# AIRI-Institute/nablaDFT

Hardware: AMD Instinct MI355X
Metric: conformer-steps/sec (fwd+bwd) + MAE(E,F) vs CPU reference (higher is better)
Workload: dtype f32 (dense products >= 192 tiles: f32 values split exactly into 3 bf16 pieces, 6 MFMA piece products, f32 accumulate; non-finite operands give NaN where plain f32 gives inf); 1 GPU; PaiNN-OC (nablaDFT/painn_pyg, config/model/painn-oc.yaml: F=128 L=6 R=100 rc=5A K=100) energy+forces train step incl. neighbour list, L1+L2 loss, grad all-reduce, clip 5.0, AdamW lr 5e-4; synthetic ~42-atom drug-like conformers, 2048 conformers/GPU/step; conformers_per_gpu=2048, edges_last_step=1737976, parallelism=dp1

## Files before the change

### include/nablaq.h

```cpp
#ifndef NABLAQ_H
#define NABLAQ_H
#include <stddef.h>
#include <stdint.h>

#ifdef __cplusplus
extern "C" {
#endif

#define NQ_OK 0
#define NQ_ERR_HIP 1
#define NQ_ERR_ARG 2
#define NQ_ERR_MOL_TOO_LARGE 3
#define NQ_ERR_WORKSPACE 4
#define NQ_ERR_NO_EDGES 5

#define NQ_ABI_VERSION 17

typedef struct nq_painn_cfg {
  int32_t hidden_channels;
  int32_t num_layers;
  int32_t num_rbf;
  int32_t num_elements;
  int32_t max_neighbors;
  int32_t envelope_exponent;
// ... 267 lines not shown
int nq_eq_layernorm_forward(const float* x, int64_t x_stride, const float* weight, const float* bias, int64_t rows, int32_t W, float eps, float* y, int64_t y_stride,
                            float* stats, void* stream);
size_t nq_eq_layernorm_scratch_floats(int64_t rows, int32_t W);
int nq_eq_layernorm_backward(const float* x, int64_t x_stride, const float* weight, const float* grad_y, int64_t g_stride, const float* stats, int64_t rows, int32_t W,
                             float* grad_x, int64_t gx_stride, float* grad_weight, float* grad_bias, float* scratch, void* stream);
int nq_eq_norm_sh_forward(const float* x, const float* w0, const float* b0, const float* affine_weight, const float* balance_weight, int64_t N, int32_t lmax,
                          int32_t C, float eps, float* y, float* stats, void* stream);
size_t nq_eq_norm_sh_scratch_floats(int64_t N, int32_t lmax, int32_t C);
int nq_eq_norm_sh_backward(const float* x, const float* w0, const float* affine_weight, const float* balance_weight, const float* grad_y, const float* stats,
                           int64_t N, int32_t lmax, int32_t C, float* grad_x, float* grad_w0, float* grad_b0, float* grad_affine_weight, float* scratch,
                           void* stream);
int nq_eq_logits_forward(const float* x, const float* alpha_dot, int64_t E, int32_t H, int32_t A, float* z, void* stream);
size_t nq_eq_logits_scratch_floats(int64_t E, int32_t H, int32_t A);
int nq_eq_logits_backward(const float* x, const float* alpha_dot, const float* grad_z, int64_t E, int32_t H, int32_t A, float* grad_x, float* grad_alpha_dot,
                          float* scratch, void* stream);
int nq_eq_softmax_forward(const float* z, const int32_t* ptr, int64_t N, int32_t H, float* out, void* stream);
int nq_eq_softmax_backward(const float* y, const float* grad_y, const int32_t* ptr, int64_t N, int32_t H, float* grad_z, void* stream);
int nq_eq_head_scale(int32_t nseg, const int32_t* rows, const float* const* x, const float* const* grad, const float* alpha, int64_t E, int32_t H, int32_t V,
                     float* const* out, float* grad_alpha, void* stream);
int nq_eq_scale(const float* x, const float* row_scale, const int32_t* row_index, const float* coef_scale, int64_t N, int32_t I, int32_t C, float* out, void* stream);

int nq_loss_l1_l2(const float* energy, const float* y, int32_t B, const float* forces, const float* f_target, int32_t N, float coef_e,
                  float coef_f, float* loss, float* grad_energy, float* grad_forces, void* stream);
int nq_loss_mse(const float* energy, const float* y, int32_t B, const float* forces, const float* f_target, int32_t N, float coef_e,
                float coef_f, float* loss, float* grad_energy, float* grad_forces, void* stream);
int nq_adamw_step(float* params, const float* grads, float* exp_avg, float* exp_avg_sq, size_t count, float max_norm, float lr,
                  float beta1, float beta2, float eps, float weight_decay, int32_t step, float* scratch, void* stream);

void nq_profile_enable(int32_t on);
int nq_profile_read(char* names_host, int32_t name_stride, double* total_ms_host, int64_t* counts_host, int32_t cap);
int nq_profile_read2(char* names_host, int32_t name_stride, double* total_ms_host, int64_t* counts_host, double* flops_host, int32_t cap);

void nq_set_gemm_variant(int32_t variant);
void nq_gemm_splitk_release(void);
int nq_gemm_splitk_state(void* stream, uint64_t* ptr, uint64_t* floats, int32_t* captured, int32_t* retired);

int nq_linear_forward(const float* A, const float* W, const float* bias, float* C, float* C_silu, int32_t M, int32_t N, int32_t K,
                      void* stream);
int nq_linear_forward_act(const float* A, const float* W, float* C, float* C_act, const float* resid, float alpha, float beta, int32_t M, int32_t N,
                          int32_t K, void* stream);
int nq_linear_forward_res(const float* A, const float* W, const float* aux, float alpha, float* C, int32_t M, int32_t N, int32_t K, void* stream);
int nq_bf16_pack(const float* W, int32_t N, int32_t K, void* Wb, void* WbT, void* stream);
int nq_linear_forward_bf16(const float* A, const void* Wb, float* C, float* C_act, const float* resid, float alpha, float beta, int32_t M, int32_t N,
                           int32_t K, void* stream);
int nq_linear_input_grad_bf16(const float* G, const void* WbT, float* C, int32_t M, int32_t N, int32_t K, int32_t accumulate, void* stream);
size_t nq_weight_grad_bf16_scratch_bytes(int64_t rows, int32_t N, int32_t K);
int nq_linear_weight_grad_bf16(const float* G, const float* X, float* gW, int64_t rows, int32_t N, int32_t K, void* scratch, void* stream);
int nq_linear_forward_bf16_out(const void* A, int32_t a_bf16, const void* Wb, void* pre_bf16, void* act, int32_t act_bf16, const float* resid, float alpha,
                               float beta, int32_t M, int32_t N, int32_t K, void* stream);
int nq_linear_weight_grad_bf16_x(const float* G, const void* X_bf16, float* gW, int64_t rows, int32_t N, int32_t K, void* scratch, void* stream);
int nq_gn_ssilu_backward_bf16(const void* z_bf16, const float* g, float scale, int64_t n, float* out, void* stream);
int nq_linear_input_grad(const float* G, const float* W, float* C, int32_t M, int32_t N, int32_t K, int32_t accumulate, void* stream);
int nq_linear_input_grad_epi(const float* G, const float* W, float* C, int32_t M, int32_t N, int32_t K, const float* aux, float alpha, float beta, int32_t mode,
                             void* stream);
int nq_linear_input_grad_bf16_epi(const float* G, const void* WbT, float* C, int32_t M, int32_t N, int32_t K, const float* aux, float alpha, float beta,
                                  int32_t mode, void* stream);
size_t nq_column_sum_scratch_floats(int64_t rows, int32_t cols);
int nq_column_sum(const float* A, int64_t rows, int32_t cols, int64_t lda, float* out, float* scratch, void* stream);
size_t nq_weight_grad_scratch_floats(int64_t rows, int32_t N, int32_t K);
int nq_linear_weight_grad(const float* G, const float* X, float* gW, int64_t rows, int32_t N, int32_t K, float* scratch, void* stream);
int nq_linear_weight_grad_bias(const float* G, const float* X, float* gW, float* gb, int64_t rows, int32_t N, int32_t K, float* scratch, void* stream);

int nq_rccl_available(void);
int nq_rccl_unique_id(void* id128);
int nq_rccl_comm_create(const void* id128, int32_t world, int32_t rank, void** comm);
int nq_rccl_comm_destroy(void* comm);
// ... 164 lines not shown
```

### nabladft_amd/_lib.py

```python
import ctypes as C
import os

import torch

_HERE = os.path.dirname(os.path.abspath(__file__))
LIB_PATH = os.environ.get("NABLAQ_LIB") or os.path.join(_HERE, "libnablaq.so")
ABI_VERSION = 17

NQ_OK, NQ_ERR_HIP, NQ_ERR_ARG, NQ_ERR_MOL_TOO_LARGE, NQ_ERR_WORKSPACE, NQ_ERR_NO_EDGES = range(6)


class NablaqError(RuntimeError):
    def __init__(self, code, msg):
        super().__init__(f"libnablaq error {code}: {msg}")
        self.code = code


class PainnCfg(C.Structure):
    _fields_ = [("hidden_channels", C.c_int32), ("num_layers", C.c_int32), ("num_rbf", C.c_int32),
                ("num_elements", C.c_int32), ("max_neighbors", C.c_int32), ("envelope_exponent", C.c_int32),
                ("cutoff", C.c_double), ("rbf_coeff", C.c_float), ("filter_mode", C.c_int32), ("rbf_type", C.c_int32), ("reserved", C.c_int32)]


class SchnetCfg(C.Structure):
# ... 134 lines not shown
    "nq_es_graph_fill": (C.c_int, [_P, _P, _P, _I32, _D, _I32, _P, _P, _P, _P, _P]),
    "nq_es_frames": (C.c_int, [_P, _I32, _P, _P]),
    "nq_es_wigner": (C.c_int, [_P, _I32, _P, _P, _P, _P, _I32, _I32, _I32, _P, _P, _P]),
    "nq_es_smearing": (C.c_int, [_P, _I64, _I32, _P, _F, _P, _P]),
    "nq_rowop": (C.c_int, [_P, _I64, _P, _I64, _P, _P, _I64, _I64, _I32, _I32, _I32, _I32, _I32, _P]),
    "nq_rowop_blocks": (C.c_int, [_P, _I64, _P, _I64, _P, _I32, _I32, _P, _P, _I64, _I32, _I32, _I32, _I32, _I32, _P]),
    "nq_s2_activation_blocks": (C.c_int, [_P, _P, _I32, _I32, _I32, _I64, _I32, _P, _P, _P, _P, _I32, _P]),
    "nq_column_sum_scratch_floats": (_SZ, [_I64, _I32]),
    "nq_column_sum": (C.c_int, [_P, _I64, _I32, _I64, _P, _P, _P]),
    "nq_es_rotate": (C.c_int, [_P, _I64, _P, _I64, _P, _I32, _P, _P, _I32, _I32, _I64, _P, _I32, _I32, _I32, _P]),
    "nq_es_rotate_back": (C.c_int, [_P, _I64, _I32, _P, _P, _I32, _I32, _P, _P, _P, _P, _I64, _P, _I32, _I32, _I32, _P]),
    "nq_eq_layernorm_forward": (C.c_int, [_P, _I64, _P, _P, _I64, _I32, _F, _P, _I64, _P, _P]),
    "nq_eq_layernorm_scratch_floats": (_SZ, [_I64, _I32]),
    "nq_eq_layernorm_backward": (C.c_int, [_P, _I64, _P, _P, _I64, _P, _I64, _I32, _P, _I64, _P, _P, _P, _P]),
    "nq_eq_norm_sh_forward": (C.c_int, [_P, _P, _P, _P, _P, _I64, _I32, _I32, _F, _P, _P, _P]),
    "nq_eq_norm_sh_scratch_floats": (_SZ, [_I64, _I32, _I32]),
    "nq_eq_norm_sh_backward": (C.c_int, [_P, _P, _P, _P, _P, _P, _I64, _I32, _I32, _P, _P, _P, _P, _P, _P]),
    "nq_eq_logits_forward": (C.c_int, [_P, _P, _I64, _I32, _I32, _P, _P]),
    "nq_eq_logits_scratch_floats": (_SZ, [_I64, _I32, _I32]),
    "nq_eq_logits_backward": (C.c_int, [_P, _P, _P, _I64, _I32, _I32, _P, _P, _P, _P]),
    "nq_eq_softmax_forward": (C.c_int, [_P, _P, _I64, _I32, _P, _P]),
    "nq_eq_softmax_backward": (C.c_int, [_P, _P, _P, _I64, _I32, _P, _P]),
    "nq_eq_head_scale": (C.c_int, [_I32, _P, _P, _P, _P, _I64, _I32, _I32, _P, _P, _P]),
    "nq_eq_scale": (C.c_int, [_P, _P, _P, _P, _I64, _I32, _I32, _P, _P]),
    "nq_loss_l1_l2": (C.c_int, [_P, _P, _I32, _P, _P, _I32, _F, _F, _P, _P, _P, _P]),
    "nq_loss_mse": (C.c_int, [_P, _P, _I32, _P, _P, _I32, _F, _F, _P, _P, _P, _P]),
    "nq_adamw_step": (C.c_int, [_P, _P, _P, _P, _SZ, _F, _F, _F, _F, _F, _F, _I32, _P, _P]),
    "nq_profile_enable": (None, [_I32]),
    "nq_profile_read": (C.c_int, [C.c_char_p, _I32, C.POINTER(C.c_double), C.POINTER(C.c_int64), _I32]),
    "nq_profile_read2": (C.c_int, [C.c_char_p, _I32, C.POINTER(C.c_double), C.POINTER(C.c_int64), C.POINTER(C.c_double), _I32]),
    "nq_set_gemm_variant": (None, [_I32]),
    "nq_gemm_splitk_release": (None, []),
    "nq_gemm_splitk_state": (C.c_int, [_P, C.POINTER(C.c_uint64), C.POINTER(C.c_uint64), C.POINTER(C.c_int32), C.POINTER(C.c_int32)]),
    "nq_linear_forward": (C.c_int, [_P, _P, _P, _P, _P, _I32, _I32, _I32, _P]),
    "nq_linear_input_grad": (C.c_int, [_P, _P, _P, _I32, _I32, _I32, _I32, _P]),
    "nq_weight_grad_scratch_floats": (_SZ, [_I64, _I32, _I32]),
    "nq_linear_weight_grad": (C.c_int, [_P, _P, _P, _I64, _I32, _I32, _P, _P]),
    "nq_linear_weight_grad_bias": (C.c_int, [_P, _P, _P, _P, _I64, _I32, _I32, _P, _P]),
    "nq_rccl_available": (C.c_int, []),
    "nq_rccl_unique_id": (C.c_int, [_P]),
    "nq_rccl_comm_create": (C.c_int, [_P, _I32, _I32, C.POINTER(C.c_void_p)]),
    "nq_rccl_comm_destroy": (C.c_int, [_P]),
    "nq_rccl_comm_count": (C.c_int, [_P, C.POINTER(C.c_int32)]),
    "nq_allreduce": (C.c_int, [_P, _SZ, _P, _P]),
    "nq_allreduce_mean": (C.c_int, [_P, _SZ, _P, _P]),
    "nq_rccl_broadcast": (C.c_int, [_P, _SZ, _I32, _P, _P]),
    "nq_lbfgs_state_bytes": (_SZ, [_I32, _I32, _I32]),
    "nq_lbfgs_state_layout": (C.c_int, [_I32, _I32, _I32, C.POINTER(_SZ)]),
    "nq_lbfgs_init": (C.c_int, [_P, _SZ, _P, _I32, _I32, _I32, _P, _I32, _P, C.POINTER(C.c_int32), _P]),
    "nq_lbfgs_step": (C.c_int, [_P, _I32, _I32, _I32, _I32, _P, _I32, _P, _P, _D, _D, _D, _D, _I32, _P]),
    "nq_md_constants": (C.c_int, [C.POINTER(C.c_double)]),
    "nq_md_state_bytes": (_SZ, [_I32, _I32, _I32, _I32, _I32]),
    "nq_md_state_layout": (C.c_int, [_I32, _I32, _I32, _I32, _I32, C.POINTER(_SZ)]),
    "nq_md_init": (C.c_int, [_P, _SZ, _P, _P, _P, _P, _I32, _I32, _I32, _I32, _I32, _P, _I32, _P, _P, C.POINTER(C.c_int32), _P]),
    "nq_md_init_velocities": (C.c_int, [_P, _I32, _I32, _I32, _I32, _I32, _I32, _D, _I64, _I32, _I32, _P]),
    "nq_md_step": (C.c_int, [_P, _I32, _I32, _I32, _I32, _I32, _I32, _P, _I32, _P, _I32, _P, _I32, _D, _D, _D, _I32, _I64, _P, _P, _I32, _P]),
    "nq_md_normals": (C.c_int, [_I64, _I32, _I32, _P, _P, _I32, _I32, _P, _P]),
    "nq_vib_state_bytes": (_SZ, [_I32, _I32, _I32, _I64]),
    "nq_vib_state_layout": (C.c_int, [_I32, _I32, _I32, _I64, C.POINTER(_SZ)]),
    "nq_vib_init": (C.c_int, [_P, _SZ, _P, _P, _P, _I32, _I32, _I32, _I64, _P, _I32, C.POINTER(C.c_int32), _P]),
    "nq_vib_displace": (C.c_int, [_P, _I32, _I32, _I32, _I64, _I32, _I32, _D, _P, _I64, _P]),
    "nq_vib_accumulate": (C.c_int, [_P, _I32, _I32, _I32, _I64, _I32, _I32, _P, _I32, _I64, _P]),
    "nq_vib_finish": (C.c_int, [_P, _I32, _I32, _I32, _I64, _P]),
    "nq_vib_eigh": (C.c_int, [_P, _I32, _I32, _I32, _I64, _I32, _I32, _I32, _I32, _P]),
    "nq_orb_state_bytes": (_SZ, [_I32, _I32, _I64]),
    "nq_orb_state_layout": (C.c_int, [_I32, _I32, _I64, C.POINTER(_SZ)]),
# ... 140 lines not shown
```

### nabladft_amd/build.py

```python
import os
import subprocess
import sys

HERE = os.path.dirname(os.path.abspath(__file__))
CSRC = os.path.join(HERE, "csrc")
OBJ = os.path.join(HERE, "csrc", "_obj")
LIB = os.path.join(HERE, "libnablaq.so")
SOURCES = ["graph.hip", "gemm.hip", "gemm_bf16.hip", "edge.hip", "molpair.hip", "updfuse.hip", "node.hip", "schnet.hip", "hblock.hip", "so3.hip", "qhnet.hip", "qhgen.hip", "gemnet_graph.hip", "gemnet.hip", "escn.hip", "equiformer.hip", "geobasis.hip", "graphormer.hip", "dimenet.hip", "lbfgs.hip", "md.hip", "vib.hip", "orbitals.hip", "orbdens.hip", "orbresp.hip", "orbsmear.hip", "orbpurify.hip", "orbbond.hip", "rccl.hip", "engine.hip"]
EXTRA = {"molpair.hip": ["-fno-slp-vectorize"], "md.hip": ["-ffp-contract=off"], "vib.hip": ["-ffp-contract=off"], "orbitals.hip": ["-ffp-contract=off"], "orbdens.hip": ["-ffp-contract=off"], "orbresp.hip": ["-ffp-contract=off"], "orbsmear.hip": ["-ffp-contract=off"], "orbpurify.hip": ["-ffp-contract=off"], "orbbond.hip": ["-ffp-contract=off"]}
FLAGS = ["--offload-arch=gfx950", "-O3", "-std=c++17", "-fPIC", "-fno-fast-math", "-ffp-contract=on", "-Wall", "-Wno-unused-function"]


def _newer(target, deps):
    if not os.path.exists(target):
        return True
    t = os.path.getmtime(target)
    return any(os.path.getmtime(d) > t for d in deps)


def build(force=False, verbose=True):
    hipcc = os.environ.get("HIPCC", "/opt/rocm/bin/hipcc")
    os.makedirs(OBJ, exist_ok=True)
    headers = [os.path.join(CSRC, "common.h"), os.path.join(CSRC, "lanes.h"), os.path.join(CSRC, "gemm_tile.h"), os.path.join(CSRC, "gemm_split.h"), os.path.join(CSRC, "cg_l4.inc"), os.path.join(CSRC, "devstate.h"), os.path.join(CSRC, "orbstate.h"), os.path.join(CSRC, "orbresp_tiles.h"), os.path.join(CSRC, "orbsmear_math.h"), os.path.join(os.path.dirname(HERE), "include", "nablaq.h")]
    objs, procs = [], []
    for s in SOURCES:
        src, obj = os.path.join(CSRC, s), os.path.join(OBJ, s.replace(".hip", ".o"))
        objs.append(obj)
        if force or _newer(obj, [src] + headers):
            cmd = [hipcc] + FLAGS + EXTRA.get(s, []) + ["-c", src, "-o", obj]
            if verbose:
                print(" ".join(cmd), flush=True)
            procs.append((s, subprocess.Popen(cmd, stdout=subprocess.PIPE, stderr=subprocess.STDOUT, text=True)))
    failed = False
    for s, p in procs:
        out, _ = p.communicate()
        if out.strip() and verbose:
            print(out)
        if p.returncode != 0:
            print(f"hipcc failed on {s}:\n{out}", file=sys.stderr)
            failed = True
    if failed:
        raise RuntimeError("hipcc compilation failed")
    if force or procs or _newer(LIB, objs):
        cmd = [hipcc, "--offload-arch=gfx950", "-shared", "-fPIC", "-o", LIB] + objs
        if verbose:
            print(" ".join(cmd), flush=True)
        subprocess.check_call(cmd)
    return LIB


if __name__ == "__main__":
    build(force="--force" in sys.argv)
    print("built", LIB)
```

### nabladft_amd/csrc/gemm.hip

```cpp
#include <algorithm>
#include <map>
#include <mutex>
#include <vector>
#include "gemm_tile.h"
#include "gemm_split.h"

#define BM 128
#define BN 128

__device__ __forceinline__ long rm_row(int q, int w, int ncomp, int base) { return (long)(q / w) * ncomp + base + q % w; }

#define LDS_KC (BM + 1)
#define LDS_MC (BM + 4)

template <bool KC, int NT, int BKT, bool MAP = false>
__device__ __forceinline__ void fetch_tile(float4 (&v)[BM * BKT / 4 / NT], const float* __restrict__ src, int ld, int r0, int R, int k0, int Kend,
                                           bool vec_ok, int mw = 1, int mn = 1, int mb = 0) {
  const int t = threadIdx.x;
#pragma unroll
  for (int it = 0; it < BM * BKT / 4 / NT; ++it) {
    const int idx = t + NT * it;
    float4 x = make_float4(0.f, 0.f, 0.f, 0.f);
    if (KC) {
      const int row = idx / (BKT / 4), kq = (idx % (BKT / 4)) * 4;
      const int gr = r0 + row, gk = k0 + kq;
      if (gr < R) {
        const float* ptr = src + (MAP ? rm_row(gr, mw, mn, mb) : (long)gr) * ld + gk;
        if (vec_ok && gk + 3 < Kend) x = *reinterpret_cast<const float4*>(ptr);
        else {
          if (gk + 0 < Kend) x.x = ptr[0];
          if (gk + 1 < Kend) x.y = ptr[1];
          if (gk + 2 < Kend) x.z = ptr[2];
          if (gk + 3 < Kend) x.w = ptr[3];
        }
      }
    } else {
      const int k = idx >> 5, rq = (idx & 31) * 4;
      const int gk = k0 + k, gr = r0 + rq;
// ... 213 lines not shown
      acc = __builtin_amdgcn_mfma_f32_32x32x2f32(a, b, acc, 0, 0, 0);
    }
    __syncthreads();
  }
  const int col = n0 + wn * 32 + lr;
  if (col >= p.N) return;
  const float bv = p.bias ? p.bias[col] : 0.f;
#pragma unroll
  for (int r = 0; r < 16; ++r) {
    const int row = m0 + wm * 32 + (r & 3) + 8 * (r >> 2) + 4 * lk;
    if (row >= p.M) continue;
    const long off = (long)row * p.ldc + col;
    const float v = acc[r] + bv;
    if (EPI == EPI_ACC) p.C[off] += v;
    else if (EPI == EPI_DSILU) p.C[off] = p.eb * v * nq_dsilu_fast(p.resid[off]);
    else if (EPI == EPI_RES) p.C[off] = p.ea * p.resid[off] + v;
    else p.C[off] = v;
    if (EPI == EPI_SILU) p.C2[off] = nq_silu(v);
    if (EPI == EPI_SILU_RES) p.C2[off] = p.resid ? p.ea * p.resid[off] + p.eb * nq_silu_fast(v) : p.eb * nq_silu_fast(v);
    if (EPI == EPI_DSILU2) p.C2[off] = v * nq_dsilu_fast(p.resid[off]);
  }
}
static bool gemm_is_small(int M, int N) { return (long)nq_cdiv(M, BM) * nq_cdiv(N, BN) < 256; }

enum GemmVariant : int {
  GV_WAVES8 = 1,
  GV_PREFETCH = 2,
  GV_NO_SMALL = 8,
  GV_GENERIC_ONLY = 16,
  GV_EXACT_F32 = 32,
  GV_SPLIT_ALWAYS = 64,
  GV_NO_SPLITK = 128,
  GV_SPH_ROW_MAPPED = 256,
};
static int g_gemm_variant = GV_WAVES8;
extern "C" void nq_set_gemm_variant(int32_t v) { g_gemm_variant = v; }

template <bool A_KC, bool B_KC, int EPI, int BKT = 32>
static void launch_gemm(hipStream_t st, dim3 grid, const GemmArgs& p) {
  int variant = g_gemm_variant & (GV_WAVES8 | GV_PREFETCH);
  if (variant == GV_WAVES8 && (long)grid.x * grid.y * grid.z < 512) variant |= GV_PREFETCH;
  if (variant == GV_WAVES8 && A_KC) variant |= GV_PREFETCH;
  switch (variant) {
    case 0: hipLaunchKernelGGL((k_gemm<A_KC, B_KC, EPI, 4, false, BKT>), grid, dim3(256), 0, st, p); break;
    case GV_WAVES8: hipLaunchKernelGGL((k_gemm<A_KC, B_KC, EPI, 8, false, BKT>), grid, dim3(512), 0, st, p); break;
    case GV_PREFETCH: hipLaunchKernelGGL((k_gemm<A_KC, B_KC, EPI, 4, true, BKT>), grid, dim3(256), 0, st, p); break;
    default: hipLaunchKernelGGL((k_gemm<A_KC, B_KC, EPI, 8, true, BKT>), grid, dim3(512), 0, st, p); break;
  }
}

#define RP_CHUNKS 8
#define RP_ELEMS 32
#define RP_MIN_SPLITS 32
__device__ __forceinline__ float reduce_range(const float* __restrict__ part, long stride, long i, int k, int kend) {
  float s0 = 0.f, s1 = 0.f, s2 = 0.f, s3 = 0.f;
  for (; k + 3 < kend; k += 4) {
    s0 += part[(long)k * stride + i]; s1 += part[(long)(k + 1) * stride + i];
    s2 += part[(long)(k + 2) * stride + i]; s3 += part[(long)(k + 3) * stride + i];
  }
  for (; k < kend; ++k) s0 += part[(long)k * stride + i];
  return (s0 + s1) + (s2 + s3);
}
__device__ __forceinline__ void reduce_partials_body(const float* __restrict__ part, int nsplit, long stride, long count, float* __restrict__ out, long block) {
  if (nsplit < RP_MIN_SPLITS) {
    const long i = block * (RP_CHUNKS * RP_ELEMS) + threadIdx.x;
    if (i < count) out[i] = reduce_range(part, stride, i, 0, nsplit);
// ... 66 lines not shown
    hipLaunchKernelGGL((k_gemm2<A_KC, B_KC, EPI, 128, 128, 32, 4, 2, 4>), dim3((unsigned)(tiles < 512 ? tiles : 512)), dim3(512), 0, st, p);
  }
}

static bool gemm3_disabled() {
  static const int env = [] { const char* e = getenv("NQ_GEMM_F32"); return (e && e[0] && e[0] != '0') ? 1 : 0; }();
  return env || (g_gemm_variant & GV_EXACT_F32);
}
bool nq_gemm_exact_f32_requested() { return gemm3_disabled(); }
template <bool A_KC, bool B_KC>
static bool gemm3_ok(const GemmArgs& p, long kspan, int splits) {
  if (gemm3_disabled() || !gemm2_ok<A_KC, B_KC>(p, kspan)) return false;
  return (g_gemm_variant & GV_SPLIT_ALWAYS) || (long)nq_cdiv(p.M, 128) * nq_cdiv(p.N, 128) * splits >= 192;
}
template <bool A_KC, bool B_KC, int EPI>
static int launch_gemm3(hipStream_t st, const GemmArgs& p, int splits) {
  constexpr bool AUX = EPI == EPI_ACC || EPI == EPI_DSILU || EPI == EPI_RES || EPI == EPI_SILU_RES || EPI == EPI_DSILU2;
  constexpr int WPE = AUX ? 2 : 3;
  const long tiles = (long)nq_cdiv(p.M, 128) * nq_cdiv(p.N, 128) * splits;
  const dim3 grid((unsigned)(tiles < 256 * WPE ? tiles : 256 * WPE));
  if constexpr (EPI == EPI_PARTIAL) {
    if (p.bpart) hipLaunchKernelGGL((k_gemm3<A_KC, B_KC, EPI, 2, false, true>), dim3((unsigned)(tiles < 512 ? tiles : 512)), dim3(256), 0, st, p);
    else hipLaunchKernelGGL((k_gemm3<A_KC, B_KC, EPI, WPE, false, false>), grid, dim3(256), 0, st, p);
  } else if (p.K & 15) {
    constexpr int WT = (A_KC && B_KC) ? WPE : 2;
    const dim3 gt((unsigned)(tiles < 256 * WT ? tiles : 256 * WT));
    hipLaunchKernelGGL((k_gemm3<A_KC, B_KC, EPI, WT, true>), gt, dim3(256), 0, st, p);
  } else {
    hipLaunchKernelGGL((k_gemm3<A_KC, B_KC, EPI, WPE, false>), grid, dim3(256), 0, st, p);
  }
  return NQ_OK;
}

template <bool A_KC, bool B_KC, int EPI, int GENERIC_BKT = 32>
static int launch_product(hipStream_t st, const GemmArgs& p, long kspan, int splits = 1) {
  constexpr bool SPLITK = A_KC && EPI == EPI_PARTIAL;
  if (gemm3_ok<A_KC, B_KC>(p, kspan, splits)) NQ_TRY((launch_gemm3<A_KC, B_KC, EPI>(st, p, splits)));
  else if (SPLITK || gemm2_ok<A_KC, B_KC>(p, kspan)) launch_gemm2<A_KC, B_KC, EPI>(st, p, splits);
  else if constexpr (!SPLITK) {
    if (A_KC && gemm_is_small(p.M, p.N) && !(g_gemm_variant & GV_NO_SMALL)) {
      if constexpr (A_KC) hipLaunchKernelGGL((k_gemm_small<B_KC, EPI>), dim3(nq_cdiv(p.M, SM), nq_cdiv(p.N, SM), 1), dim3(256), 0, st, p);
    } else {
      launch_gemm<A_KC, B_KC, EPI, GENERIC_BKT>(st, dim3(nq_cdiv(p.M, BM), nq_cdiv(p.N, BN), splits), p);
    }
  }
  NQ_LAUNCH_CHECK();
  return NQ_OK;
}

template <bool A_KC, bool B_KC, int EPI>
static bool launch_batched(hipStream_t st, const GemmArgs& p, int splits, long kspan) {
  if (g_gemm_variant & GV_SPH_ROW_MAPPED) return false;
  if (!gemm2_ok<A_KC, B_KC>(p, kspan) || p.nbatch < 1) return false;
  if ((p.bsA & 3) || (p.bsB & 3) || (p.bsC & 3) || (p.ldc & 3) || (reinterpret_cast<uintptr_t>(p.C) & 15)) return false;
  if (p.bz) for (int L = 0; L < 7; ++L) if (p.Bz[L] && (reinterpret_cast<uintptr_t>(p.Bz[L]) & 15)) return false;
  const long t128 = (long)nq_cdiv(p.M, 128) * nq_cdiv(p.N, 128) * splits, t64 = (long)nq_cdiv(p.M, 64) * nq_cdiv(p.N, 64) * splits;
  const bool use3 = !gemm3_disabled() && !p.bpart && EPI != EPI_PARTIAL && ((g_gemm_variant & GV_SPLIT_ALWAYS) || t128 * p.nbatch >= 192) && !(p.K & 15);
  if (use3) {
    const long cap = 256 * 3;
    const unsigned gx = (unsigned)std::min<long>(t128, std::max<long>(1, (cap + p.nbatch - 1) / p.nbatch));
    hipLaunchKernelGGL((k_gemm3<A_KC, B_KC, EPI, 3, false, false, NQ_GEMM3_TERMS, 0, true>), dim3(gx, p.nbatch), dim3(256), 0, st, p);
  } else if (gemm2_small_tiles(p.M * p.nbatch, p.N, splits)) {
    const unsigned gx = (unsigned)std::min<long>(t64, std::max<long>(1, (1024 + p.nbatch - 1) / p.nbatch));
    hipLaunchKernelGGL((k_gemm2<A_KC, B_KC, EPI, 64, 64, 32, 2, 2, 4, 0, true>), dim3(gx, p.nbatch), dim3(256), 0, st, p);
  } else {
    const unsigned gx = (unsigned)std::min<long>(t128, std::max<long>(1, (512 + p.nbatch - 1) / p.nbatch));
    hipLaunchKernelGGL((k_gemm2<A_KC, B_KC, EPI, 128, 128, 32, 4, 2, 4, 0, true>), dim3(gx, p.nbatch), dim3(512), 0, st, p);
  }
  return true;
// ... 282 lines not shown
    GemmArgs b = p;
    b.M = (int)rows; b.lda = ncomp * K; b.ldc = ncomp * N; b.nbatch = ncomp; b.bz = 1; b.bsA = K; b.bsB = 0; b.bsC = N;
    if (launch_batched<true, B_KC, EPI_STORE>(st, b, 1, K)) { NQ_LAUNCH_CHECK(); return NQ_OK; }
  }
  dim3 grid(nq_cdiv(p.M, BM), nq_cdiv(N, BN), order + 1);
  hipLaunchKernelGGL((k_gemm<true, B_KC, EPI_STORE, 8, true, B_KC ? 32 : 16, 1>), grid, dim3(512), 0, st, p);
  NQ_LAUNCH_CHECK();
  return NQ_OK;
}

extern "C" {

int nq_linear_forward(const float* A, const float* Wt, const float* bias, float* C, float* C_silu, int32_t M, int32_t N, int32_t K, void* stream) {
  return nq_gemm_nt((hipStream_t)stream, A, Wt, C, bias, C_silu, M, N, K, K, K, N);
}
int nq_linear_forward_act(const float* A, const float* Wt, float* C, float* C_act, const float* resid, float alpha, float beta, int32_t M, int32_t N, int32_t K,
                          void* stream) {
  if (!A || !Wt || !C || !C_act) return nq_fail(NQ_ERR_ARG, "null argument");
  return nq_gemm_nt_act((hipStream_t)stream, A, Wt, C, C_act, resid, alpha, beta, M, N, K);
}
int nq_linear_forward_res(const float* A, const float* Wt, const float* aux, float alpha, float* C, int32_t M, int32_t N, int32_t K, void* stream) {
  if (!A || !Wt || !C || !aux) return nq_fail(NQ_ERR_ARG, "null argument");
  if (aux == C) return nq_fail(NQ_ERR_ARG, "nq_linear_forward_res: aux must not alias C");
  return nq_gemm_nt_res((hipStream_t)stream, A, Wt, C, aux, alpha, M, N, K);
}
int nq_linear_input_grad(const float* G, const float* Wt, float* C, int32_t M, int32_t N, int32_t K, int32_t accumulate, void* stream) {
  return nq_gemm_nn((hipStream_t)stream, G, Wt, C, M, N, K, N, K, K, accumulate);
}
int nq_linear_input_grad_epi(const float* G, const float* Wt, float* C, int32_t M, int32_t N, int32_t K, const float* aux, float alpha, float beta, int32_t mode,
                             void* stream) {
  if (!G || !Wt || !C || !aux || (mode != 1 && mode != 2)) return nq_fail(NQ_ERR_ARG, "bad argument");
  return nq_gemm_nn_epi((hipStream_t)stream, G, Wt, C, M, N, K, aux, alpha, beta, mode);
}
size_t nq_column_sum_scratch_floats(int64_t rows, int32_t cols) { return nq_colsum_scratch_floats((long)rows, cols); }
int nq_column_sum(const float* A, int64_t rows, int32_t cols, int64_t lda, float* out, float* scratch, void* stream) {
  if (!A || !out || !scratch || cols < 1 || lda < cols) return nq_fail(NQ_ERR_ARG, "column_sum: bad argument");
  return nq_colsum((hipStream_t)stream, A, (long)rows, cols, (int)lda, out, scratch);
}
size_t nq_weight_grad_scratch_floats(int64_t rows, int32_t N, int32_t K) { return nq_gemm_tn_scratch_floats(rows, N, K); }
int nq_linear_weight_grad(const float* G, const float* X, float* gW, int64_t rows, int32_t N, int32_t K, float* scratch, void* stream) {
  return nq_gemm_tn((hipStream_t)stream, G, X, gW, rows, N, K, N, K, scratch);
}
int nq_linear_weight_grad_bias(const float* G, const float* X, float* gW, float* gb, int64_t rows, int32_t N, int32_t K, float* scratch, void* stream) {
  if (!gb) return nq_fail(NQ_ERR_ARG, "null bias gradient");
  return nq_gemm_tn((hipStream_t)stream, G, X, gW, rows, N, K, N, K, scratch, nullptr, gb, rows);
}

int nq_sph_linear_forward(const float* x, const float* const* W_host, const float* bias0, float* y, int64_t rows, int32_t order, int32_t Fin,
                          int32_t Fout, void* stream) {
  return sph_linear<true>(x, W_host, bias0, y, rows, order, Fin, Fout, "sph_linear_fwd", (hipStream_t)stream);
}

int nq_sph_linear_input_grad(const float* gy, const float* const* W_host, float* gx, int64_t rows, int32_t order, int32_t Fin, int32_t Fout,
                             void* stream) {
  return sph_linear<false>(gy, W_host, nullptr, gx, rows, order, Fin, Fout, "sph_linear_bwd_x", (hipStream_t)stream);
}

size_t nq_sph_weight_grad_scratch_floats(int64_t rows, int32_t order, int32_t Fin, int32_t Fout) {
  const size_t ncomp = (size_t)(order + 1) * (order + 1);
  const size_t sps = sph_tn_splits(rows, (int)ncomp);
  const size_t part = ncomp * sps * (size_t)Fout * Fin + sps * (size_t)Fout, cs = nq_colsum_scratch_floats(rows, Fout);
  return part > cs ? part : cs;
}

int nq_sph_linear_weight_grad(const float* gy, const float* x, float* const* gW_host, float* gbias0, int64_t rows, int32_t order, int32_t Fin,
                              int32_t Fout, float* scratch, void* stream) {
// ... 49 lines not shown
```

Baseline: 52640 conformer-steps/s.

## Add persistent B-resident split-bf16 GEMM kernel for small-K products

Adds a persistent GEMM kernel that splits a 128-column block of the weight matrix into three bf16 planes once and keeps it resident in LDS. Each wave then streams 32-row A tiles through a double-buffered per-wave stage with buffer loads and runs the split-precision MFMA products against the resident B. It is used when K is at most 128, K is a multiple of 16, and there are at least two column blocks. The goal is to stop re-loading and re-splitting B for every output tile and to cut launch and tile overhead on tall, skinny products. The trade-offs are high LDS use that limits occupancy, per-wave synchronisation, and a fixed grid sized for 256 CUs; a probe entry point and a planning query are also added.

```diff
diff --git a/include/nablaq.h b/include/nablaq.h
--- a/include/nablaq.h
+++ b/include/nablaq.h
@@ -323,6 +323,9 @@
 int nq_profile_read2(char* names_host, int32_t name_stride, double* total_ms_host, int64_t* counts_host, double* flops_host, int32_t cap);
 
 void nq_set_gemm_variant(int32_t variant);
+int nq_gemm_resident_plan(int64_t M, int64_t N, int64_t K, int32_t nbatch, int32_t* out4);
+int nq_gemm_probe(int32_t layout, int32_t epi, const float* A, const float* W, float* C, float* C2, const float* bias, const float* aux, float alpha, float beta,
+                  int32_t M, int32_t N, int32_t K, int32_t lda, int32_t ldw, int32_t ldc, void* stream);
 void nq_gemm_splitk_release(void);
 int nq_gemm_splitk_state(void* stream, uint64_t* ptr, uint64_t* floats, int32_t* captured, int32_t* retired);
 
diff --git a/nabladft_amd/_lib.py b/nabladft_amd/_lib.py
--- a/nabladft_amd/_lib.py
+++ b/nabladft_amd/_lib.py
@@ -190,6 +190,8 @@
     "nq_set_gemm_variant": (None, [_I32]),
     "nq_gemm_splitk_release": (None, []),
     "nq_gemm_splitk_state": (C.c_int, [_P, C.POINTER(C.c_uint64), C.POINTER(C.c_uint64), C.POINTER(C.c_int32), C.POINTER(C.c_int32)]),
+    "nq_gemm_resident_plan": (C.c_int, [_I64, _I64, _I64, _I32, C.POINTER(C.c_int32)]),
+    "nq_gemm_probe": (C.c_int, [_I32, _I32, _P, _P, _P, _P, _P, _P, _F, _F, _I32, _I32, _I32, _I32, _I32, _I32, _P]),
     "nq_linear_forward": (C.c_int, [_P, _P, _P, _P, _P, _I32, _I32, _I32, _P]),
     "nq_linear_input_grad": (C.c_int, [_P, _P, _P, _I32, _I32, _I32, _I32, _P]),
     "nq_weight_grad_scratch_floats": (_SZ, [_I64, _I32, _I32]),
diff --git a/nabladft_amd/build.py b/nabladft_amd/build.py
--- a/nabladft_amd/build.py
+++ b/nabladft_amd/build.py
@@ -21,7 +21,7 @@
 def build(force=False, verbose=True):
     hipcc = os.environ.get("HIPCC", "/opt/rocm/bin/hipcc")
     os.makedirs(OBJ, exist_ok=True)
-    headers = [os.path.join(CSRC, "common.h"), os.path.join(CSRC, "lanes.h"), os.path.join(CSRC, "gemm_tile.h"), os.path.join(CSRC, "gemm_split.h"), os.path.join(CSRC, "cg_l4.inc"), os.path.join(CSRC, "devstate.h"), os.path.join(CSRC, "orbstate.h"), os.path.join(CSRC, "orbresp_tiles.h"), os.path.join(CSRC, "orbsmear_math.h"), os.path.join(os.path.dirname(HERE), "include", "nablaq.h")]
+    headers = [os.path.join(CSRC, "common.h"), os.path.join(CSRC, "lanes.h"), os.path.join(CSRC, "gemm_tile.h"), os.path.join(CSRC, "gemm_split.h"), os.path.join(CSRC, "gemm_resident.h"), os.path.join(CSRC, "gemm_resident_plan.h"), os.path.join(CSRC, "cg_l4.inc"), os.path.join(CSRC, "devstate.h"), os.path.join(CSRC, "orbstate.h"), os.path.join(CSRC, "orbresp_tiles.h"), os.path.join(CSRC, "orbsmear_math.h"), os.path.join(os.path.dirname(HERE), "include", "nablaq.h")]
     objs, procs = [], []
     for s in SOURCES:
         src, obj = os.path.join(CSRC, s), os.path.join(OBJ, s.replace(".hip", ".o"))
diff --git a/nabladft_amd/csrc/gemm.hip b/nabladft_amd/csrc/gemm.hip
--- a/nabladft_amd/csrc/gemm.hip
+++ b/nabladft_amd/csrc/gemm.hip
@@ -4,6 +4,7 @@
 #include <vector>
 #include "gemm_tile.h"
 #include "gemm_split.h"
+#include "gemm_resident.h"
 
 #define BM 128
 #define BN 128
@@ -283,6 +284,7 @@
   GV_SPLIT_ALWAYS = 64,
   GV_NO_SPLITK = 128,
   GV_SPH_ROW_MAPPED = 256,
+  GV_NO_RESIDENT = 512,
 };
 static int g_gemm_variant = GV_WAVES8;
 extern "C" void nq_set_gemm_variant(int32_t v) { g_gemm_variant = v; }
@@ -415,9 +417,37 @@
   return NQ_OK;
 }
 
+template <bool A_KC, bool B_KC, int EPI>
+static bool gemm3r_plan(const GemmArgs& p, long kspan, int splits, ResidentPlan& pl) {
+  return resident_plan(pl, p.M, p.N, p.K, A_KC, p.nbatch, EPI == EPI_PARTIAL, gemm3_ok<A_KC, B_KC>(p, kspan, splits), (g_gemm_variant & GV_NO_RESIDENT) != 0);
+}
+template <bool B_KC, int EPI>
+static int launch_gemm3r(hipStream_t st, const GemmArgs& p, const ResidentPlan& pl) {
+  static_assert(RES_MAX_K <= 144, "a 64-column flavour would be needed");
+  if (pl.nc != 128) return nq_fail(NQ_ERR_ARG, "resident product: no flavour for this column block");
+  const auto k = k_gemm3r<B_KC, EPI, 128>;
+  NQ_DYN_LDS(k, (size_t)pl.lds_bytes);
+  hipLaunchKernelGGL(k, dim3((unsigned)pl.gx, (unsigned)pl.gy), dim3(RES_WAVES * 64), (size_t)pl.lds_bytes, st, p);
+  return NQ_OK;
+}
+extern "C" int nq_gemm_resident_plan(int64_t M, int64_t N, int64_t K, int32_t nbatch, int32_t* out4) {
+  ResidentPlan pl;
+  const bool ok = resident_plan(pl, (long)M, (long)N, (long)K, true, nbatch, false, !gemm3_disabled(), (g_gemm_variant & GV_NO_RESIDENT) != 0);
+  if (out4) { out4[0] = pl.nc; out4[1] = pl.lds_bytes; out4[2] = pl.gx; out4[3] = pl.gy; }
+  return ok ? 1 : 0;
+}
+
 template <bool A_KC, bool B_KC, int EPI, int GENERIC_BKT = 32>
 static int launch_product(hipStream_t st, const GemmArgs& p, long kspan, int splits = 1) {
   constexpr bool SPLITK = A_KC && EPI == EPI_PARTIAL;
+  if constexpr (A_KC && EPI != EPI_PARTIAL) {
+    ResidentPlan pl;
+    if (gemm3r_plan<A_KC, B_KC, EPI>(p, kspan, splits, pl)) {
+      NQ_TRY((launch_gemm3r<B_KC, EPI>(st, p, pl)));
+      NQ_LAUNCH_CHECK();
+      return NQ_OK;
+    }
+  }
   if (gemm3_ok<A_KC, B_KC>(p, kspan, splits)) NQ_TRY((launch_gemm3<A_KC, B_KC, EPI>(st, p, splits)));
   else if (SPLITK || gemm2_ok<A_KC, B_KC>(p, kspan)) launch_gemm2<A_KC, B_KC, EPI>(st, p, splits);
   else if constexpr (!SPLITK) {
@@ -766,6 +796,29 @@
   if (!G || !Wt || !C || !aux || (mode != 1 && mode != 2)) return nq_fail(NQ_ERR_ARG, "bad argument");
   return nq_gemm_nn_epi((hipStream_t)stream, G, Wt, C, M, N, K, aux, alpha, beta, mode);
 }
+int nq_gemm_probe(int32_t layout, int32_t epi, const float* A, const float* W, float* C, float* C2, const float* bias, const float* aux, float ea, float eb,
+                  int32_t M, int32_t N, int32_t K, int32_t lda, int32_t ldw, int32_t ldc, void* stream) {
+  if (!A || !W || !C || M < 1 || N < 1 || K < 1 || lda < K || ldc < N || ldw < (layout ? N : K)) return nq_fail(NQ_ERR_ARG, "gemm_probe: bad argument");
+  const bool two = epi == EPI_SILU || epi == EPI_SILU_RES || epi == EPI_DSILU2, reads = epi == EPI_DSILU || epi == EPI_RES || epi == EPI_DSILU2;
+  if ((two && !C2) || (reads && !aux)) return nq_fail(NQ_ERR_ARG, "gemm_probe: the epilogue needs C2 / aux");
+  hipStream_t st = (hipStream_t)stream;
+  GemmArgs p = gemm_args(A, W, C, M, N, K, lda, ldw, ldc);
+  p.bias = bias; p.C2 = C2; gemm_aux(p, aux, ea, eb);
+  if (layout == 0) switch (epi) {
+    case EPI_STORE: return launch_product<true, true, EPI_STORE>(st, p, K);
+    case EPI_SILU: return launch_product<true, true, EPI_SILU>(st, p, K);
+    case EPI_SILU_RES: return launch_product<true, true, EPI_SILU_RES>(st, p, K);
+    case EPI_DSILU2: return launch_product<true, true, EPI_DSILU2>(st, p, K);
+    case EPI_RES: return launch_product<true, true, EPI_RES>(st, p, K);
+  } else if (layout == 1) switch (epi) {
+    case EPI_STORE: return launch_product<true, false, EPI_STORE, 16>(st, p, K);
+    case EPI_ACC: return launch_product<true, false, EPI_ACC, 16>(st, p, K);
+    case EPI_DSILU: return launch_product<true, false, EPI_DSILU, 16>(st, p, K);
+    case EPI_RES: return launch_product<true, false, EPI_RES, 16>(st, p, K);
+    case EPI_DSILU2: return launch_product<true, false, EPI_DSILU2, 16>(st, p, K);
+  }
+  return nq_fail(NQ_ERR_ARG, "gemm_probe: no launcher of this layout reaches this epilogue");
+}
 size_t nq_column_sum_scratch_floats(int64_t rows, int32_t cols) { return nq_colsum_scratch_floats((long)rows, cols); }
 int nq_column_sum(const float* A, int64_t rows, int32_t cols, int64_t lda, float* out, float* scratch, void* stream) {
   if (!A || !out || !scratch || cols < 1 || lda < cols) return nq_fail(NQ_ERR_ARG, "column_sum: bad argument");
diff --git a/nabladft_amd/csrc/gemm_resident.h b/nabladft_amd/csrc/gemm_resident.h
--- /dev/null
+++ b/nabladft_amd/csrc/gemm_resident.h
@@ -0,0 +1,169 @@
+#pragma once
+#include "gemm_split.h"
+#include "gemm_resident_plan.h"
+
+struct ResStageA {
+  static constexpr int ROWS = RES_ROWS, PITCH = 32, PLANE = ROWS * PITCH, BYTES = 3 * PLANE;
+
+  static __device__ __forceinline__ __amdgpu_buffer_rsrc_t descriptor(const float* __restrict__ A, long lda, int m0, int M, int K) {
+    const float* base = A + (long)m0 * lda;
+    const long rr = min(M - m0, ROWS);
+    const long bytes = ((rr - 1) * lda + K) * 4;
+    const unsigned long long b = reinterpret_cast<unsigned long long>(base);
+    const unsigned lo = __builtin_amdgcn_readfirstlane((unsigned)b), hi = __builtin_amdgcn_readfirstlane((unsigned)(b >> 32));
+    const int nrec = __builtin_amdgcn_readfirstlane((int)max(0L, min(bytes, 0xffffffffL)));
+    return __builtin_amdgcn_make_buffer_rsrc(reinterpret_cast<float*>(((unsigned long long)hi << 32) | lo), 0, rr > 0 ? nrec : 0, 0x00020000);
+  }
+  static __device__ __forceinline__ int lane_offset(int lda, int lane) { return ((lane >> 1) * lda + (lane & 1) * 8) * 4; }
+  static __device__ __forceinline__ void fetch(float (&v)[8], __amdgpu_buffer_rsrc_t rsrc, int voff, int k0_) {
+    const int k0 = __builtin_amdgcn_readfirstlane(k0_);
+    const gemm_u32x4 x = __builtin_amdgcn_raw_buffer_load_b128(rsrc, voff, k0 * 4, 0), y = __builtin_amdgcn_raw_buffer_load_b128(rsrc, voff, k0 * 4 + 16, 0);
+    v[0] = __uint_as_float(x.x); v[1] = __uint_as_float(x.y); v[2] = __uint_as_float(x.z); v[3] = __uint_as_float(x.w);
+    v[4] = __uint_as_float(y.x); v[5] = __uint_as_float(y.y); v[6] = __uint_as_float(y.z); v[7] = __uint_as_float(y.w);
+  }
+  static __device__ __forceinline__ void stash(char* __restrict__ tile, const float (&v)[8], int lane) {
+    unsigned h[4], m[4], l[4];
+#pragma unroll
+    for (int e = 0; e < 4; ++e) sp_split2(v[2 * e], v[2 * e + 1], h[e], m[e], l[e]);
+    char* q = tile + (lane >> 1) * PITCH + (lane & 1) * 16;
+    *reinterpret_cast<gemm_u32x4*>(q) = gemm_u32x4{h[0], h[1], h[2], h[3]};
+    *reinterpret_cast<gemm_u32x4*>(q + PLANE) = gemm_u32x4{m[0], m[1], m[2], m[3]};
+    *reinterpret_cast<gemm_u32x4*>(q + 2 * PLANE) = gemm_u32x4{l[0], l[1], l[2], l[3]};
+  }
+  static __device__ __forceinline__ sp_bf8 frag(const char* __restrict__ tile, int pl, int lr, int lk) {
+    return *reinterpret_cast<const sp_bf8*>(tile + pl * PLANE + lr * PITCH + lk * 16);
+  }
+};
+
+__device__ __forceinline__ void res_wave_sync() {
+  __builtin_amdgcn_fence(__ATOMIC_RELEASE, "wavefront");
+  __builtin_amdgcn_wave_barrier();
+  __builtin_amdgcn_fence(__ATOMIC_ACQUIRE, "wavefront");
+}
+
+struct ResStep { int rt, k0; };
+
+template <bool B_KC, int EPI, int NC, int NW = RES_WAVES, int PD = 2, int TERMS = NQ_GEMM3_TERMS>
+__global__ __launch_bounds__(NW * 64, NW / 4) void k_gemm3r(GemmArgs p) {
+  static_assert(EPI != EPI_PARTIAL && NC % 32 == 0 && PD % 2 == 0 && NW % 4 == 0, "bad flavour");
+  constexpr int TN = NC / 32, BPLANE = NC * 32, BSTEP = 3 * BPLANE;
+  constexpr bool AUX = EPI == EPI_ACC || EPI == EPI_DSILU || EPI == EPI_RES || EPI == EPI_SILU_RES || EPI == EPI_DSILU2;
+  using SA = ResStageA;
+  extern __shared__ __attribute__((aligned(16))) char res_lds[];
+  char* const Bres = res_lds + NW * 2 * SA::BYTES;
+
+  const int lane = threadIdx.x & 63, wave = __builtin_amdgcn_readfirstlane((int)(threadIdx.x >> 6));
+  const int lr = lane & 31, lk = lane >> 5;
+  const int n0 = blockIdx.y * NC;
+
+  {
+    const int koct = p.K >> 3, items = NC * koct;
+    for (int idx = threadIdx.x; idx < items; idx += NW * 64) {
+      const int r = B_KC ? idx / koct : idx % NC, ko = B_KC ? idx % koct : idx / NC;
+      float x[8];
+#pragma unroll
+      for (int e = 0; e < 8; ++e) x[e] = 0.f;
+      if (n0 + r < p.N) {
+        if (B_KC) {
+          const float4* q = reinterpret_cast<const float4*>(p.B + (long)(n0 + r) * p.ldb + ko * 8);
+          const float4 a = q[0], b = q[1];
+          x[0] = a.x; x[1] = a.y; x[2] = a.z; x[3] = a.w; x[4] = b.x; x[5] = b.y; x[6] = b.z; x[7] = b.w;
+        } else {
+          const float* q = p.B + (long)(ko * 8) * p.ldb + n0 + r;
+#pragma unroll
+          for (int e = 0; e < 8; ++e) x[e] = q[(long)e * p.ldb];
+        }
+      }
+      unsigned h[4], m[4], l[4];
+#pragma unroll
+      for (int e = 0; e < 4; ++e) sp_split2(x[2 * e], x[2 * e + 1], h[e], m[e], l[e]);
+      char* q = Bres + (ko >> 1) * BSTEP + r * 32 + (ko & 1) * 16;
+      *reinterpret_cast<gemm_u32x4*>(q) = gemm_u32x4{h[0], h[1], h[2], h[3]};
+      *reinterpret_cast<gemm_u32x4*>(q + BPLANE) = gemm_u32x4{m[0], m[1], m[2], m[3]};
+      *reinterpret_cast<gemm_u32x4*>(q + 2 * BPLANE) = gemm_u32x4{l[0], l[1], l[2], l[3]};
+    }
+  }
+  __syncthreads();
+
+  const int ntm = (p.M + SA::ROWS - 1) / SA::ROWS, stride = (int)gridDim.x * NW;
+  char* const Aw = res_lds + wave * 2 * SA::BYTES;
+  const int voff = SA::lane_offset(p.lda, lane);
+  auto first_step = [&](int rt) { return ResStep{rt, 0}; };
+  auto advance = [&](const ResStep& s) {
+    if (s.rt < ntm && s.k0 + 16 < p.K) return ResStep{s.rt, s.k0 + 16};
+    return first_step(s.rt >= ntm ? s.rt : s.rt + stride);
+  };
+  auto descriptor = [&](const ResStep& s) { return SA::descriptor(p.A, p.lda, s.rt < ntm ? s.rt * SA::ROWS : p.M, p.M, p.K); };
+
+  f32x16 acc[TN];
+#pragma unroll
+  for (int j = 0; j < TN; ++j)
+#pragma unroll
+    for (int r = 0; r < 16; ++r) acc[j][r] = 0.f;
+
+  ResStep st[PD + 1];
+  st[0] = first_step((int)blockIdx.x * NW + wave);
+#pragma unroll
+  for (int i = 1; i <= PD; ++i) st[i] = advance(st[i - 1]);
+  float ra[PD][8];
+#pragma unroll
+  for (int i = 0; i < PD; ++i) SA::fetch(ra[i], descriptor(st[i]), voff, st[i].k0);
+  SA::stash(Aw, ra[0], lane);
+  res_wave_sync();
+  do {
+#pragma unroll
+    for (int u = 0; u < PD; ++u) {
+      const ResStep cur = st[0];
+      const char* As = Aw + (u & 1) * SA::BYTES;
+      const char* Bs = Bres + (cur.k0 >> 4) * BSTEP;
+      const int m0 = cur.rt * SA::ROWS;
+      const bool last_k = cur.rt < ntm && cur.k0 + 16 >= p.K;
+      const long tile_off = (long)m0 * p.ldc + n0;
+      const bool full = m0 + SA::ROWS <= p.M && n0 + NC <= p.N;
+      float bias_v[TN];
+      f32x16 aux[AUX ? TN : 1];
+      if (last_k) {
+        const __amdgpu_buffer_rsrc_t dbias = __builtin_amdgcn_make_buffer_rsrc(const_cast<float*>(p.bias), 0, p.bias ? p.N * 4 : 0, 0x00020000);
+#pragma unroll
+        for (int j = 0; j < TN; ++j) bias_v[j] = __uint_as_float(__builtin_amdgcn_raw_buffer_load_b32(dbias, (n0 + j * 32 + lr) * 4, 0, 0));
+        if (AUX) {
+          const __amdgpu_buffer_rsrc_t daux = gemm_aux_descriptor(EPI == EPI_ACC ? p.C : p.resid, tile_off, (long)(p.M - 1) * p.ldc + p.N);
+#pragma unroll
+          for (int j = 0; j < TN; ++j) gemm_load_aux(aux[AUX ? j : 0], daux, p.ldc, 4 * lk, j * 32 + lr);
+        }
+      }
+      SA::fetch(ra[u], descriptor(st[PD]), voff, st[PD].k0);
+      {
+        sp_bf8 fa[3], fb[3][TN];
+#pragma unroll
+        for (int pl = 0; pl < 3; ++pl) {
+          fa[pl] = SA::frag(As, pl, lr, lk);
+#pragma unroll
+          for (int j = 0; j < TN; ++j) fb[pl][j] = *reinterpret_cast<const sp_bf8*>(Bs + pl * BPLANE + (j * 32 + lr) * 32 + lk * 16);
+        }
+        constexpr int PA[9] = {2, 2, 1, 1, 2, 0, 1, 0, 0}, PB[9] = {2, 1, 2, 1, 0, 2, 0, 1, 0};
+#pragma unroll
+        for (int tt = 9 - TERMS; tt < 9; ++tt)
+#pragma unroll
+          for (int j = 0; j < TN; ++j) acc[j] = __builtin_amdgcn_mfma_f32_32x32x16_bf16(fa[PA[tt]], fb[PB[tt]][j], acc[j], 0, 0, 0);
+      }
+      SA::stash(Aw + ((u & 1) ^ 1) * SA::BYTES, ra[(u + 1) % PD], lane);
+      if (last_k) {
+        __builtin_amdgcn_s_waitcnt(0x0F70 | 2);
+        float* tbase = p.C + tile_off;
+#pragma unroll
+        for (int j = 0; j < TN; ++j) {
+          const int rl = 4 * lk, cl = j * 32 + lr;
+          if (full) gemm_store_acc<EPI, true>(acc[j], aux[AUX ? j : 0], p, tbase, rl, cl, SA::ROWS, NC, bias_v[j], tile_off);
+          else gemm_store_acc<EPI, false>(acc[j], aux[AUX ? j : 0], p, tbase, rl, cl, p.M - m0, p.N - n0, bias_v[j], tile_off);
+#pragma unroll
+          for (int r = 0; r < 16; ++r) acc[j][r] = 0.f;
+        }
+      }
+#pragma unroll
+      for (int i = 0; i < PD; ++i) st[i] = st[i + 1];
+      st[PD] = advance(st[PD]);
+      res_wave_sync();
+    }
+  } while (st[0].rt < ntm);
+}
diff --git a/nabladft_amd/csrc/gemm_resident_plan.h b/nabladft_amd/csrc/gemm_resident_plan.h
--- /dev/null
+++ b/nabladft_amd/csrc/gemm_resident_plan.h
@@ -0,0 +1,44 @@
+#pragma once
+
+#define RES_WAVES 8
+#define RES_ROWS 32
+#define RES_A_BYTES (RES_WAVES * 2 * 3 * RES_ROWS * 32)
+#define RES_LDS_BUDGET (160 * 1024)
+#define RES_CUS 256
+#define RES_MAX_K 128
+#define RES_MIN_BLOCKS 2
+
+struct ResidentPlan {
+  int nc;
+  int lds_bytes;
+  int gx, gy;
+};
+
+static inline long resident_plane_bytes(int nc, int K) { return 6L * nc * K; }
+
+static inline int resident_column_block(int K) {
+  if (K <= 0) return 0;
+  for (int nc = 128; nc >= 64; nc >>= 1)
+    if (resident_plane_bytes(nc, K) + RES_A_BYTES <= RES_LDS_BUDGET) return nc;
+  return 0;
+}
+
+static inline bool resident_plan(ResidentPlan& pl, long M, long N, long K, bool a_kc, int nbatch, bool partial, bool on_split_engine, bool switched_off,
+                                 int max_k = RES_MAX_K, int min_blocks = RES_MIN_BLOCKS) {
+  pl = ResidentPlan{0, 0, 0, 0};
+  if (switched_off || !on_split_engine || !a_kc || partial || nbatch > 1) return false;
+  if (M <= 0 || N <= 0 || K <= 0 || (K & 15) || K > max_k || M > 0x7fffffffL - RES_ROWS || N > 0x7fffffffL - 128) return false;
+  const int nc = resident_column_block((int)K);
+  if (!nc) return false;
+  const long ncb = (N + nc - 1) / nc;
+  if (ncb > 65535 || ncb < min_blocks) return false;
+  const long row_tiles = (M + RES_ROWS - 1) / RES_ROWS, chunks = (row_tiles + RES_WAVES - 1) / RES_WAVES;
+  long gx = RES_CUS / ncb;
+  if (gx < 1) gx = 1;
+  if (gx > chunks) gx = chunks;
+  pl.nc = nc;
+  pl.lds_bytes = (int)(resident_plane_bytes(nc, (int)K) + RES_A_BYTES);
+  pl.gx = (int)gx;
+  pl.gy = (int)ncb;
+  return true;
+}
```

After: 52950 conformer-steps/s, median of 5. About the same (+0.6%).
